# earth-insights/ZoomEarth

Measured on AMD Instinct MI355X. Metric: questions/sec end-to-end, ZoomEarth-3B on 5000px tiles, higher is better.
Workload: dtype bf16

## Files before the change

zoomearth_amd/csrc/ze_attention.hip:

```cpp
#include "ze_kernels.h"

typedef __attribute__((ext_vector_type(8))) __bf16 bf16x8;
typedef __attribute__((ext_vector_type(4))) float f32x4;

#define FA_BQ 64
#ifndef ZE_FA_CAUSAL_BKV
#define ZE_FA_CAUSAL_BKV 64
#endif
#define FA_BK 64

typedef short v4s __attribute__((ext_vector_type(4)));
typedef unsigned int fa_u32x4 __attribute__((ext_vector_type(4)));

__device__ __forceinline__ uint32_t fa_pack_bf16(float lo, float hi) {
    typedef __attribute__((ext_vector_type(2))) float fa_f32x2_;
    typedef __attribute__((ext_vector_type(2))) __bf16 fa_bf16x2_;
    const fa_bf16x2_ b = __builtin_convertvector(fa_f32x2_{lo, hi}, fa_bf16x2_);
    uint32_t r;
    __builtin_memcpy(&r, &b, 4);
    return r;
}

__device__ __forceinline__ int fa_off(int row, int ch) { return 256 * row + 16 * (ch ^ ze_kv_swz(row)); }

template <int D, int CAUSAL, int BKV, int QT = 1, bool DMA = false>
__global__ void __launch_bounds__(256) __attribute__((amdgpu_waves_per_eu(2))) k_flash_attn(const bf16_t* __restrict__ q, int q_rs, int q_hs,
                                                    const bf16_t* __restrict__ k, int k_rs, int k_hs,
                                                    const bf16_t* __restrict__ v, int v_rs, int v_hs,
                                                    bf16_t* __restrict__ o, int o_rs, int o_hs,
                                                    const int4* __restrict__ tiles, int group, float scale_log2e,
                                                    int q_pos_offset, const int* __restrict__ tile_aux,
                                                    size_t kv_seq_stride, ze_fa_rope rope) {
    constexpr int KS = (D + 31) / 32;
    constexpr int DCH = D / 8;
    constexpr int NV = D / 16;
    extern __shared__ __attribute__((aligned(16))) uint8_t smem[];
    constexpr int TILE_B = BKV * 256, NKT = BKV / 16, RP = BKV / 64;

    const int4 tile = tiles[blockIdx.x];
    const int q0 = tile.x, q1 = tile.y, kv0 = tile.z, kv1 = tile.w;
    if (tile_aux) {
        k += (size_t)tile_aux[2 * blockIdx.x] * kv_seq_stride;
        v += (size_t)tile_aux[2 * blockIdx.x] * kv_seq_stride;
        q_pos_offset = tile_aux[2 * blockIdx.x + 1];
    }
    const int head = blockIdx.y, kvh = head / group;
    const int tid = threadIdx.x, lane = tid & 63, wid = tid >> 6;
    const int fr = lane & 15, fq = lane >> 4;
    int qi[QT];
#pragma unroll
    for (int t = 0; t < QT; ++t) qi[t] = q0 + (wid * QT + t) * 16 + fr;

    bf16x8 qf[QT][KS];
#pragma unroll
    for (int t = 0; t < QT; ++t)
#pragma unroll
        for (int ks = 0; ks < KS; ++ks) {
            uint4 val = make_uint4(0, 0, 0, 0);
            const int ch = ks * 4 + fq;
            if (qi[t] < q1 && ch < DCH) val = *reinterpret_cast<const uint4*>(q + (size_t)qi[t] * q_rs + (size_t)head * q_hs + ch * 8);
            qf[t][ks] = *reinterpret_cast<const bf16x8*>(&val);
        }

    f32x4 oacc[QT][NV];
    float m_run[QT], l_run[QT];
#pragma unroll
    for (int t = 0; t < QT; ++t) {
#pragma unroll
        for (int j = 0; j < NV; ++j) oacc[t][j] = f32x4{0.f, 0.f, 0.f, 0.f};
        m_run[t] = -INFINITY;
        l_run[t] = 0.f;
    }
    int kv_hi = kv1;
    if (CAUSAL) kv_hi = min(kv1, q1 + q_pos_offset);
    const int ntile = (kv_hi - kv0 + BKV - 1) / BKV;

    const int srow = tid >> 2, sch = (tid & 3) * 4;
    fa_u32x4 rk[RP][4], rv[RP][4];
    auto stage_load = [&](int kt) {
#pragma unroll
        for (int rp = 0; rp < RP; ++rp) {
            const int keyc = min(kt + rp * 64 + srow, kv_hi - 1);
            const bf16_t* kp = k + (size_t)keyc * k_rs + (size_t)kvh * k_hs;
            const bf16_t* vp = v + (size_t)keyc * v_rs + (size_t)kvh * v_hs;
#pragma unroll
            for (int i = 0; i < 4; ++i) {
                const int ch = min(sch + i, DCH - 1);
                rk[rp][i] = *reinterpret_cast<const fa_u32x4*>(kp + ch * 8);
                rv[rp][i] = *reinterpret_cast<const fa_u32x4*>(vp + ch * 8);
            }
        }
    };
    auto stage_write = [&](int buf, int kt) {
        uint8_t* kb = smem + buf * 2 * TILE_B;
#pragma unroll
        for (int rp = 0; rp < RP; ++rp) {
            const bool ok = kt + rp * 64 + srow < kv_hi;
#pragma unroll
            for (int i = 0; i < 4; ++i) {
                const unsigned m = (ok && (sch + i < DCH)) ? 0xffffffffu : 0u;
                *reinterpret_cast<fa_u32x4*>(kb + fa_off(rp * 64 + srow, sch + i)) = rk[rp][i] & m;
                *reinterpret_cast<fa_u32x4*>(kb + TILE_B + fa_off(rp * 64 + srow, sch + i)) = rv[rp][i] & m;
            }
        }
    };
    static_assert(!DMA || (D == 128 && BKV == 64), "the LDS-DMA staging moves whole 256-byte rows of 64-key tiles");
    const unsigned smem_lds = __builtin_amdgcn_readfirstlane((unsigned)(size_t)(__attribute__((address_space(3))) uint8_t*)smem);
    const int wid_u = __builtin_amdgcn_readfirstlane(wid);
    auto stage_dma = [&](int buf, int kt) {
        const unsigned kimg = smem_lds + (unsigned)buf * 2u * TILE_B, vimg = kimg + TILE_B;
        const int r4 = lane >> 4, pos = lane & 15;
#pragma unroll
        for (int g = 0; g < 4; ++g) {
            const int pc = wid_u * 4 + g;
            const int row = 4 * pc + r4;
            const int ch = pos ^ ze_kv_swz(row);
            const int keyc = min(kt + row, kv_hi - 1);
            const bf16_t* ksrc = k + (size_t)keyc * k_rs + (size_t)kvh * k_hs + ch * 8;
            const bf16_t* vsrc = v + (size_t)keyc * v_rs + (size_t)kvh * v_hs + ch * 8;
            unsigned keep;
            asm volatile(
                "s_mov_b32 %0, m0\n\ts_mov_b32 m0, %3\n\ts_nop 0\n\tglobal_load_lds_dwordx4 %1, off\n\t"
                "s_mov_b32 m0, %4\n\ts_nop 0\n\tglobal_load_lds_dwordx4 %2, off\n\ts_mov_b32 m0, %0"
                : "=&s"(keep)
                : "v"(ksrc), "v"(vsrc), "s"(kimg + (unsigned)pc * 1024u), "s"(vimg + (unsigned)pc * 1024u)
                : "memory");
        }
    };
    if (ntile > 0) {
        if constexpr (DMA) stage_dma(0, kv0);
        else stage_load(kv0);
    }
    if constexpr (D == 128) {
        if (rope.cosT) {
#pragma unroll
            for (int t = 0; t < QT; ++t)
                if (qi[t] < q1) {
#pragma unroll
                    for (int ks = 0; ks < 2; ++ks) {
                        const int j = ks * 32 + fq * 8;
                        const int axis = j < rope.s0 ? 0 : (j < rope.s01 ? 1 : 2);
                        const int pos = rope.pos3[axis * rope.T + qi[t]];
                        const uint4 c4 = *reinterpret_cast<const uint4*>(rope.cosT + (size_t)pos * 64 + j);
                        const uint4 s4 = *reinterpret_cast<const uint4*>(rope.sinT + (size_t)pos * 64 + j);
                        uint4 o1, o2;
                        rope8(*reinterpret_cast<const uint4*>(&qf[t][ks]), *reinterpret_cast<const uint4*>(&qf[t][ks + 2]), c4, s4, o1, o2);
                        qf[t][ks] = *reinterpret_cast<const bf16x8*>(&o1);
                        qf[t][ks + 2] = *reinterpret_cast<const bf16x8*>(&o2);
                    }
                }
        }
    }

    if (ntile > 0) {
        if constexpr (DMA) asm volatile("s_waitcnt vmcnt(0)" ::: "memory");
        else stage_write(0, kv0);
    }
    __syncthreads();

    for (int t = 0; t < ntile; ++t) {
        const int kt = kv0 + t * BKV;
        const uint8_t* kb = smem + (t & 1) * 2 * TILE_B;
        const uint8_t* vb = kb + TILE_B;
        if (t + 1 < ntile) {
            if constexpr (DMA) stage_dma((t + 1) & 1, kt + BKV);
            else stage_load(kt + BKV);
        }
        f32x4 sacc[QT][NKT];
#pragma unroll
        for (int u = 0; u < QT; ++u)
#pragma unroll
            for (int n = 0; n < NKT; ++n) sacc[u][n] = f32x4{0.f, 0.f, 0.f, 0.f};
#pragma unroll
        for (int ks = 0; ks < KS; ++ks) {
#pragma unroll
            for (int n = 0; n < NKT; ++n) {
                const uint4 ka = *reinterpret_cast<const uint4*>(kb + fa_off(n * 16 + fr, ks * 4 + fq));
#pragma unroll
                for (int u = 0; u < QT; ++u)
                    sacc[u][n] = __builtin_amdgcn_mfma_f32_16x16x32_bf16(*reinterpret_cast<const bf16x8*>(&ka), qf[u][ks], sacc[u][n],
                                                                        0, 0, 0);
            }
        }
        uint32_t pw[QT][NKT][2];
#pragma unroll
        for (int u = 0; u < QT; ++u) {
            float p[NKT][4];
// ... 53 lines not shown
                }
            }
#pragma unroll
            for (int n = 0; n < NKT; ++n) {
                pw[u][n][0] = fa_pack_bf16(p[n][0], p[n][1]);
                pw[u][n][1] = fa_pack_bf16(p[n][2], p[n][3]);
            }
        }
#pragma unroll
        for (int ks = 0; ks < BKV / 32; ++ks) {
            bf16x8 pb[QT];
#pragma unroll
            for (int u = 0; u < QT; ++u) {
                const uint4 pq = make_uint4(pw[u][2 * ks][0], pw[u][2 * ks][1], pw[u][2 * ks + 1][0], pw[u][2 * ks + 1][1]);
                pb[u] = *reinterpret_cast<const bf16x8*>(&pq);
            }
#pragma unroll
            for (int j = 0; j < NV; ++j) {
                const int l16 = lane & 15, tq = l16 >> 2, tp = l16 & 3;
                const int r0a = ks * 32 + fq * 4, r0b = r0a + 16;
                const int ch = j * 2 + (tp >> 1), half = 8 * (tp & 1);
                const v4s lo = __builtin_amdgcn_ds_read_tr16_b64_v4i16(
                    (__attribute__((address_space(3))) v4s*)(vb + fa_off(r0a + tq, ch) + half));
                const v4s hi = __builtin_amdgcn_ds_read_tr16_b64_v4i16(
                    (__attribute__((address_space(3))) v4s*)(vb + fa_off(r0b + tq, ch) + half));
                typedef short v8s __attribute__((ext_vector_type(8)));
                const v8s va = __builtin_shufflevector(lo, hi, 0, 1, 2, 3, 4, 5, 6, 7);
#pragma unroll
                for (int u = 0; u < QT; ++u)
                    oacc[u][j] = __builtin_amdgcn_mfma_f32_16x16x32_bf16(*reinterpret_cast<const bf16x8*>(&va), pb[u], oacc[u][j], 0, 0, 0);
            }
        }
        if constexpr (DMA) asm volatile("s_waitcnt vmcnt(0)" ::: "memory");
        else if (t + 1 < ntile) stage_write((t + 1) & 1, kt + BKV);
        __syncthreads();
    }
#pragma unroll
    for (int u = 0; u < QT; ++u)
        if (qi[u] < q1) {
            const float inv = l_run[u] > 0.f ? 1.0f / l_run[u] : 0.f;
#pragma unroll
            for (int j = 0; j < NV; ++j) {
                uint2 w;
                w.x = pack_bf16x2(oacc[u][j][0] * inv, oacc[u][j][1] * inv);
                w.y = pack_bf16x2(oacc[u][j][2] * inv, oacc[u][j][3] * inv);
                *reinterpret_cast<uint2*>(o + (size_t)qi[u] * o_rs + (size_t)head * o_hs + j * 16 + fq * 4) = w;
            }
        }
}

void ze_launch_flash_attn(int D, int causal, const bf16_t* q, int q_rs, int q_hs, const bf16_t* k, int k_rs,
                          int k_hs, const bf16_t* v, int v_rs, int v_hs, bf16_t* o, int o_rs, int o_hs,
                          const int4* tiles, int n_tiles, int heads, int group, float scale, int q_pos_offset,
                          hipStream_t s, const int* tile_aux, size_t kv_seq_stride, int q_tile, int max_kv, ze_fa_rope rope) {
    if (n_tiles == 0) return;
    const float sl = scale * 1.4426950408889634f;
    dim3 grid(n_tiles, heads);
#define FA_LAUNCH_(DD, CC, QQ, DM)                                                                                 \
    do {                                                                                                          \
        constexpr int BKV_ = (CC) ? ZE_FA_CAUSAL_BKV : 64;                                                        \
        constexpr int LDS_ = 4 * BKV_ * 256;                                                                      \
        static bool attr_set = false;                                                                             \
        if (!attr_set) {                                                                                          \
            hipFuncSetAttribute(reinterpret_cast<const void*>(&k_flash_attn<DD, CC, BKV_, QQ, DM>),               \
                                hipFuncAttributeMaxDynamicSharedMemorySize, LDS_);                                \
            attr_set = true;                                                                                      \
        }                                                                                                         \
        const int lds_ = (max_kv > 0 && max_kv <= BKV_) ? LDS_ / 2 : LDS_;                                        \
        hipLaunchKernelGGL((k_flash_attn<DD, CC, BKV_, QQ, DM>), grid, dim3(256), lds_, s, q, q_rs, q_hs, k, k_rs, k_hs, v, v_rs, \
                           v_hs, o, o_rs, o_hs, tiles, group, sl, q_pos_offset, tile_aux, kv_seq_stride, rope);    \
    } while (0)
#define FA_LAUNCH(DD, CC, QQ) FA_LAUNCH_(DD, CC, QQ, false)
    if (D == 128 && causal && ZE_FA_CAUSAL_BKV == 64 && ze_knobs[ZE_KNOB_GATE_UP_FLASH] != ZE_FLASH_REG_STAGED && k_rs % 8 == 0 && v_rs % 8 == 0 && k_hs % 8 == 0 &&
        v_hs % 8 == 0 && ((size_t)k % 16) == 0 && ((size_t)v % 16) == 0 && kv_seq_stride % 8 == 0) {
        if (q_tile > 64) FA_LAUNCH_(128, 1, 2, true);
        else FA_LAUNCH_(128, 1, 1, true);
        return;
    }
    if (q_tile > 64) {
        if (D == 80) {
            if (causal) FA_LAUNCH(80, 1, 2); else FA_LAUNCH(80, 0, 2);
        } else {
            if (causal) FA_LAUNCH(128, 1, 2); else FA_LAUNCH(128, 0, 2);
        }
        return;
    }
    if (D == 80) {
        if (causal) FA_LAUNCH(80, 1, 1); else FA_LAUNCH(80, 0, 1);
    } else {
        if (causal) FA_LAUNCH(128, 1, 1); else FA_LAUNCH(128, 0, 1);
    }
#undef FA_LAUNCH
#undef FA_LAUNCH_
}
```

zoomearth_amd/csrc/ze_elementwise.hip:

```cpp
#include <hip/hip_fp16.h>

#include "ze_kernels.h"
#include "ze_prng.h"
#include "ze_rmsnorm.h"

__device__ __forceinline__ int map_row(int r, int mode, int offset) {
    return mode == 0 ? offset + r : (r >> 4) * 32 + (r & 15) + offset;
}

__global__ void __launch_bounds__(256) k_pack_rows(const void* __restrict__ src, int dtype, int row0, int nrows,
                                                   int cols, bf16_t* __restrict__ dst, int ld, int mode, int offset) {
    const size_t i = (size_t)blockIdx.x * 256 + threadIdx.x;
    if (i >= (size_t)nrows * cols) return;
    const int r = (int)(i / cols), c = (int)(i % cols);
    bf16_t v;
    if (dtype == ZE_BF16) {
        v = ((const bf16_t*)src)[i];
    } else if (dtype == ZE_F16) {
        v = f32_to_bf16(__half2float(((const __half*)src)[i]));
    } else {
        v = f32_to_bf16(((const float*)src)[i]);
    }
    dst[(size_t)map_row(row0 + r, mode, offset) * ld + c] = v;
}

__global__ void __launch_bounds__(256) k_fill_rows(uint64_t seed, float c_scale, float base, int rows, int cols,
                                                   bf16_t* __restrict__ dst, int ld, int mode, int offset) {
    const size_t i = (size_t)blockIdx.x * 256 + threadIdx.x;
    if (i >= (size_t)rows * cols) return;
    const int r = (int)(i / cols), c = (int)(i % cols);
    const float v = (c_scale != 0.0f) ? base + ze_normal_ih4(seed, i, c_scale) : base;
    dst[(size_t)map_row(r, mode, offset) * ld + c] = f32_to_bf16(v);
}

void ze_launch_pack_rows(const void* src, int dtype, int row0, int nrows, int cols, bf16_t* dst, int ld, int mode,
// ... 190 lines not shown
    }
    const uint2 v = *reinterpret_cast<const uint2*>(W + (size_t)row * ld8 + ks * 32 + (lane >> 4) * 8);
    *reinterpret_cast<uint2*>(Wf + (frag * 64 + lane) * 8) = v;
}
void ze_launch_pack_fragments8(const uint8_t* W8, int ld8, int n, int k, uint8_t* Wf8, hipStream_t s, int rope_dim) {
    const size_t frags = (size_t)((n + 15) >> 4) * (k >> 5);
    if (frags == 0) return;
    k_pack_fragments8<<<(unsigned)((frags + 3) / 4), 256, 0, s>>>(W8, ld8, n, k, Wf8, rope_dim);
}

void ze_launch_pack_fragments(const bf16_t* W, int ldw, int n, int k, bf16_t* Wf, hipStream_t s, int rope_dim) {
    const size_t frags = (size_t)((n + 15) >> 4) * (k >> 5);
    if (frags == 0) return;
    k_pack_fragments<<<(unsigned)((frags + 3) / 4), 256, 0, s>>>(W, ldw, n, k, Wf, rope_dim);
}

__global__ void __launch_bounds__(256) k_gather_cast_rows(const float* __restrict__ src, int k,
                                                          const int* __restrict__ perm, bf16_t* __restrict__ dst,
                                                          int kp, int rows) {
    const size_t i = (size_t)blockIdx.x * 256 + threadIdx.x;
    if (i >= (size_t)rows * kp) return;
    const int r = (int)(i / kp), c = (int)(i % kp);
    const int sr = perm ? perm[r] : r;
    dst[i] = c < k ? f32_to_bf16(src[(size_t)sr * k + c]) : (bf16_t)0;
}
void ze_launch_gather_cast_rows(const float* src, int k, const int* perm, bf16_t* dst, int kp, int rows,
                                hipStream_t s) {
    const size_t n = (size_t)rows * kp;
    if (n == 0) return;
    k_gather_cast_rows<<<(unsigned)((n + 255) / 256), 256, 0, s>>>(src, k, perm, dst, kp, rows);
}

__global__ void __launch_bounds__(256) k_vision_rope(bf16_t* __restrict__ qkv, const float* __restrict__ cosT,
                                                     const float* __restrict__ sinT, int n, int heads, int D) {
    const int half = D >> 1;
    const size_t i = (size_t)blockIdx.x * 256 + threadIdx.x;
    const size_t total = (size_t)n * 2 * heads * half;
    if (i >= total) return;
    const int j = (int)(i % half);
    const int hh = (int)((i / half) % heads);
    const int which = (int)((i / ((size_t)half * heads)) % 2);
    const int row = (int)(i / ((size_t)half * heads * 2));
    bf16_t* p = qkv + (((size_t)row * 3 + which) * heads + hh) * D;
    const float c = cosT[(size_t)row * half + j], s = sinT[(size_t)row * half + j];
    const float x1 = bf16_to_f32(p[j]), x2 = bf16_to_f32(p[j + half]);
    p[j] = f32_to_bf16(__fadd_rn(__fmul_rn(x1, c), __fmul_rn(-x2, s)));
    p[j + half] = f32_to_bf16(__fadd_rn(__fmul_rn(x2, c), __fmul_rn(x1, s)));
}
__global__ void __launch_bounds__(256) k_vision_rope_vec(bf16_t* __restrict__ qkv, const float* __restrict__ cosT,
                                                         const float* __restrict__ sinT, int n, int heads, int D) {
    const int half = D >> 1, hv = half >> 3;
    const size_t i = (size_t)blockIdx.x * 256 + threadIdx.x;
    const size_t total = (size_t)n * 2 * heads * hv;
    if (i >= total) return;
    const int j = (int)(i % hv) * 8;
    const int hh = (int)((i / hv) % heads);
    const int which = (int)((i / ((size_t)hv * heads)) % 2);
    const int row = (int)(i / ((size_t)hv * heads * 2));
    bf16_t* p = qkv + (((size_t)row * 3 + which) * heads + hh) * D;
    const uint4 a = *reinterpret_cast<const uint4*>(p + j), b = *reinterpret_cast<const uint4*>(p + j + half);
    const float4 c0 = *reinterpret_cast<const float4*>(cosT + (size_t)row * half + j);
    const float4 c1 = *reinterpret_cast<const float4*>(cosT + (size_t)row * half + j + 4);
    const float4 s0 = *reinterpret_cast<const float4*>(sinT + (size_t)row * half + j);
    const float4 s1 = *reinterpret_cast<const float4*>(sinT + (size_t)row * half + j + 4);
    const float cs[8] = {c0.x, c0.y, c0.z, c0.w, c1.x, c1.y, c1.z, c1.w};
    const float sn[8] = {s0.x, s0.y, s0.z, s0.w, s1.x, s1.y, s1.z, s1.w};
    const uint32_t* pa = reinterpret_cast<const uint32_t*>(&a);
    const uint32_t* pb = reinterpret_cast<const uint32_t*>(&b);
    uint32_t r1[4], r2[4];
#pragma unroll
    for (int q = 0; q < 4; ++q) {
        const float x1l = __uint_as_float(pa[q] << 16), x1h = __uint_as_float(pa[q] & 0xffff0000u);
        const float x2l = __uint_as_float(pb[q] << 16), x2h = __uint_as_float(pb[q] & 0xffff0000u);
        const uint32_t l1 = f32_to_bf16(__fadd_rn(__fmul_rn(x1l, cs[2 * q]), __fmul_rn(-x2l, sn[2 * q])));
        const uint32_t h1 = f32_to_bf16(__fadd_rn(__fmul_rn(x1h, cs[2 * q + 1]), __fmul_rn(-x2h, sn[2 * q + 1])));
        const uint32_t l2 = f32_to_bf16(__fadd_rn(__fmul_rn(x2l, cs[2 * q]), __fmul_rn(x1l, sn[2 * q])));
        const uint32_t h2 = f32_to_bf16(__fadd_rn(__fmul_rn(x2h, cs[2 * q + 1]), __fmul_rn(x1h, sn[2 * q + 1])));
        r1[q] = l1 | (h1 << 16);
        r2[q] = l2 | (h2 << 16);
    }
    *reinterpret_cast<uint4*>(p + j) = make_uint4(r1[0], r1[1], r1[2], r1[3]);
    *reinterpret_cast<uint4*>(p + j + half) = make_uint4(r2[0], r2[1], r2[2], r2[3]);
}
void ze_launch_vision_rope(bf16_t* qkv, const float* cosT, const float* sinT, int n, int heads, int D,
                           hipStream_t s) {
    const size_t total = (size_t)n * 2 * heads * (D / 2);
    if (total == 0) return;
    if ((D / 2) % 8 == 0 && ((size_t)qkv % 16) == 0) {
        const size_t tv = total / 8;
        k_vision_rope_vec<<<(unsigned)((tv + 255) / 256), 256, 0, s>>>(qkv, cosT, sinT, n, heads, D);
        return;
    }
    k_vision_rope<<<(unsigned)((total + 255) / 256), 256, 0, s>>>(qkv, cosT, sinT, n, heads, D);
}

int ze_mrope_vec_ok = 1;
#define mrope_vec_ok (ze_mrope_vec_ok != 0)


__global__ void __launch_bounds__(256) k_mrope_kv(bf16_t* __restrict__ qkv, int T, int heads, int kv_heads, int D,
                                                  const bf16_t* __restrict__ cosT, const bf16_t* __restrict__ sinT,
                                                  const int* __restrict__ pos3, const int* __restrict__ axis_of,
                                                  bf16_t* __restrict__ kcache, bf16_t* __restrict__ vcache,
                                                  int max_ctx, int past, const int* __restrict__ row_aux,
                                                  size_t cache_seq_stride) {
    const int half = D >> 1;
    const int nh = heads + 2 * kv_heads;
    const size_t i = (size_t)blockIdx.x * 256 + threadIdx.x;
    const size_t total = (size_t)T * nh * half;
    if (i >= total) return;
    const int j = (int)(i % half);
    const int hh = (int)((i / half) % nh);
    const int t = (int)(i / ((size_t)half * nh));
    int cpos = past + t;
    if (row_aux) {
        kcache += (size_t)row_aux[2 * t] * cache_seq_stride;
        vcache += (size_t)row_aux[2 * t] * cache_seq_stride;
        cpos = row_aux[2 * t + 1];
    }
    bf16_t* p = qkv + (size_t)t * nh * D + (size_t)hh * D;
    if (hh >= heads + kv_heads) {
        const int kvh = hh - heads - kv_heads;
        bf16_t* d = vcache + ((size_t)kvh * max_ctx + cpos) * D;
        d[j] = p[j];
        d[j + half] = p[j + half];
        return;
// ... 268 lines not shown
```

zoomearth_amd/csrc/ze_kernels.h:

```cpp
#pragma once
#include "ze_common.h"
#include "ze_knobs.h"

enum { ZE_EPI_NONE = 0, ZE_EPI_GELU = 1, ZE_EPI_RESIDUAL = 2, ZE_EPI_SWIGLU = 3, ZE_EPI_F32 = 4, ZE_EPI_QKV_ROPE = 5 };
enum { ZE_GV_QKV_ROPE = 0, ZE_GV_RESIDUAL = 1, ZE_GV_SWIGLU = 2, ZE_GV_LOGITS = 3, ZE_GV_PLAIN = 4 };

#if defined(__HIPCC__)
__device__ __forceinline__ int ze_kv_swz(int row) {
#ifdef ZE_KV_SWZ_OLD
    return ((row & 3) << 2) | ((row >> 2) & 3);
#else
    const int hi = (row >> 3) & 1;
    return ((((row & 7) ^ (hi << 2)) << 1) | hi);
#endif
}
#endif

#if defined(__HIPCC__)
__device__ __forceinline__ void rope8(const uint4& a, const uint4& b, const uint4& c4, const uint4& s4, uint4& o1, uint4& o2) {
    const uint32_t* pa = reinterpret_cast<const uint32_t*>(&a);
    const uint32_t* pb = reinterpret_cast<const uint32_t*>(&b);
    const uint32_t* pc = reinterpret_cast<const uint32_t*>(&c4);
    const uint32_t* ps = reinterpret_cast<const uint32_t*>(&s4);
    uint32_t r1[4], r2[4];
// ... 48 lines not shown
void ze_launch_fill_rows(uint64_t seed, float c_scale, float base, int rows, int cols, bf16_t* dst, int ld, int mode,
                         int offset, hipStream_t s);
struct ze_gemm_ws {
    float* slab = nullptr;
    size_t slab_floats = 0;
    unsigned* tickets = nullptr;
    int ticket_cap = 0;
};
void ze_launch_rmsnorm(const bf16_t* x, int ldx, const bf16_t* w, bf16_t* y, int ldy, int rows, int cols, float eps,
                       hipStream_t s, int frag = 0, int act8 = 0, uint8_t* y8 = nullptr, float* yscale = nullptr);
void ze_launch_pack_fragments(const bf16_t* W, int ldw, int n, int k, bf16_t* Wf, hipStream_t s, int rope_dim = 0);
void ze_launch_gemm_oneshot(int epi, const bf16_t* Xf, const bf16_t* Wf, const bf16_t* bias, const bf16_t* R, int ldr,
                            bf16_t* C, int ldc, int M, int N, int K, hipStream_t s, const float* wscale = nullptr,
                            const float* ascale = nullptr,
                            const uint8_t* wscale4 = nullptr);
void ze_launch_qkv_rope_oneshot(const bf16_t* Xf, const bf16_t* Wf_perm, const bf16_t* bias, bf16_t* q_out, int ldq, int M,
                                int K, int heads, int kv_heads, const bf16_t* cosT, const bf16_t* sinT,
                                const ze_seq_dev* st, const int* seq_ids, bf16_t* kcache, bf16_t* vcache,
                                size_t cache_seq_stride, int max_ctx, hipStream_t s, const float* wscale = nullptr,
                                const float* ascale = nullptr,
                                const int* row_off = nullptr,
                                const uint8_t* wscale4 = nullptr);
bool ze_launch_gemm_mx(int epi, const uint8_t* A, int lda, const float* sa, const uint8_t* W, int ldw, const float* sw,
                       const bf16_t* bias, bf16_t* C, int ldc, int M, int N, int K, hipStream_t s);
void ze_launch_gemm_frag(int epi, const bf16_t* Xf, const bf16_t* Wf, const bf16_t* bias, const bf16_t* R, int ldr,
                         bf16_t* C, int ldc, int M, int N, int K, hipStream_t s, const float* wscale = nullptr,
                         const float* ascale = nullptr,
                         const uint8_t* wscale4 = nullptr);
void ze_launch_pack_fragments8(const uint8_t* W8, int ld8, int n, int k, uint8_t* Wf8, hipStream_t s, int rope_dim = 0);
void ze_launch_pack_fragments4(const uint8_t* q4, const uint8_t* scale, int n, int k, uint8_t* Wf4, uint8_t* Sf4, hipStream_t s,
                               int rope_dim = 0);
void ze_launch_gather_cast_rows(const float* src, int k, const int* perm, bf16_t* dst, int kp, int rows,
                                hipStream_t s);
void ze_launch_vision_rope(bf16_t* qkv, const float* cosT, const float* sinT, int n, int heads, int D, hipStream_t s);
void ze_launch_mrope_kv(bf16_t* qkv, int T, int heads, int kv_heads, int D, const bf16_t* cosT, const bf16_t* sinT,
                        const int* pos3, const int* axis_of, bf16_t* kcache, bf16_t* vcache, int max_ctx, int past, const int* row_aux, size_t cache_seq_stride,
                        hipStream_t s, int q_skip = 0);
extern int ze_mrope_vec_ok;
void ze_launch_embed_rows(const int* src, const bf16_t* embed, const bf16_t* image_embeds, bf16_t* out, int T,
                          int hidden, hipStream_t s);
void ze_launch_scatter_rows(const bf16_t* src, int lds_, const int* dst_idx, bf16_t* dst, int ldd, int rows, int cols,
                            hipStream_t s);

struct ze_qkv_epi {
    const ze_seq_dev* st;
    const int* seq_ids;
    const bf16_t* cosT;
    const bf16_t* sinT;
    bf16_t* kcache;
    bf16_t* vcache;
    size_t cache_seq_stride;
    int max_ctx, heads, kv_heads, pad_;
};
void ze_launch_permute_qkv(const bf16_t* W, int ldw, const bf16_t* bias, int n_heads_total, int K, bf16_t* Wp, bf16_t* bias_p, hipStream_t s);
void ze_launch_gemm_qkv_rope(const bf16_t* A, int lda, const bf16_t* Wp, int ldw, const bf16_t* bias_p, const ze_qkv_epi* dev_args,
                             bf16_t* C, int ldc, int M, int N, int K, hipStream_t s);

void ze_launch_gemm(int epi, const bf16_t* A, int lda, const bf16_t* W, int ldw, const bf16_t* bias, const bf16_t* R,
                    int ldr, bf16_t* C, int ldc, const int* c_rows, int M, int N, int K, hipStream_t s, const ze_gemm_ws& ws = ze_gemm_ws());

void ze_launch_gemm_stream(int epi, const bf16_t* A, int lda, const bf16_t* W, int ldw, const bf16_t* bias,
                           const bf16_t* R, int ldr, bf16_t* C, int ldc, int M, int N, int K, const ze_gemm_ws& ws,
                           hipStream_t s);
void ze_launch_gemm_wide(int epi, const bf16_t* A, int lda, const bf16_t* W, int ldw, const bf16_t* bias, const bf16_t* R,
                         int ldr, bf16_t* C, int ldc, int M, int N, int K, const ze_gemm_ws& ws, hipStream_t s);

void ze_launch_gemm_p8(int epi, const bf16_t* A, int lda, const bf16_t* W, int ldw, const bf16_t* bias, const bf16_t* R, int ldr,
// ... 8 lines not shown
    const bf16_t* bias;
    bf16_t* out_bf16;
    float* out_f32;
    const ze_seq_dev* st;
    const bf16_t* cosT;
    const bf16_t* sinT;
    bf16_t* kcache;
    bf16_t* vcache;
    int heads, kv_heads, D, max_ctx;
    const bf16_t* embed;
    bf16_t* embed_out;
    const uint8_t* W8;
    const float* scale8;
    int ldw8;
    int act8;
    const uint8_t* seen;
    float penalty;
    float* amax_ws;
    const uint8_t* W4;
    const uint8_t* scale4;
};
bool ze_launch_gemv(int epi, const ze_gemv_args& a, hipStream_t s);
bool ze_launch_logits_rows(const bf16_t* W, int ldw, int N, int K, const bf16_t* norm_w, float eps, const bf16_t* const* x_rows,
                           float* const* out_rows, int n, hipStream_t s);
void ze_launch_quantize_rows(bf16_t* w, int rows, int cols, int ld, uint8_t* q, int ld8, float* scale, hipStream_t s);
void ze_launch_quantize_mxfp4(bf16_t* w, int rows, int cols, int ld, uint8_t* q, uint8_t* scale, hipStream_t s);

struct ze_fa_rope {
    const bf16_t* cosT;
    const bf16_t* sinT;
    const int* pos3;
    int s0, s01;
    int T;
};
void ze_launch_flash_attn(int D, int causal, const bf16_t* q, int q_row_stride, int q_head_stride, const bf16_t* k,
                          int k_row_stride, int k_head_stride, const bf16_t* v, int v_row_stride, int v_head_stride,
                          bf16_t* o, int o_row_stride, int o_head_stride, const int4* tiles, int n_tiles, int heads,
                          int group, float scale, int q_pos_offset, hipStream_t s, const int* tile_aux = nullptr,
                          size_t kv_seq_stride = 0, int q_tile = 64, int max_kv = 0, ze_fa_rope rope = ze_fa_rope{nullptr, nullptr, nullptr, 0, 0, 0});
#define ZE_FA_BQ_LONG 128
void ze_launch_attn_decode(const bf16_t* q, int q_row_stride, const bf16_t* kcache, const bf16_t* vcache,
                           size_t cache_seq_stride, bf16_t* out, int out_row_stride, const ze_seq_dev* st,
                           const int* seq_ids, int n, int heads, int kv_heads, int D, int max_ctx, float scale,
                           float* ws_partial, int max_splits, unsigned* tickets, hipStream_t s);

void ze_launch_attn_decode_stream(const bf16_t* q, int q_row_stride, const bf16_t* kcache, const bf16_t* vcache,
                                  size_t cache_seq_stride, bf16_t* out, int out_row_stride, const ze_seq_dev* st,
                                  const int* seq_ids, int n, int heads, int kv_heads, int max_ctx, float scale,
                                  float* ws_partial, int max_parts, unsigned* tickets, hipStream_t s, int chunk = 0,
                                  int per_wave = 0,
                                  const int* prefix = nullptr,
                                  const int* mate = nullptr, int long_parts = 0, int use_split = 0);
void ze_launch_attn_decode_rows(const bf16_t* q, int q_row_stride, const bf16_t* kcache, const bf16_t* vcache, size_t cache_seq_stride,
                                bf16_t* out, int out_row_stride, const ze_seq_dev* st, const int* seq_ids, const int* row_off, int n, int heads,
                                int kv_heads, int max_ctx, float scale, float* ws_partial, unsigned* tickets, int parts, const int* prefix,
                                hipStream_t s);

void ze_launch_kv_copy_prefix(bf16_t* kcache, bf16_t* vcache, size_t layer_stride, size_t seq_stride, size_t head_stride,
                              int layers, int kv_heads, int D, int src, int dst, int n_tokens, hipStream_t s);
void ze_launch_kv_fork(bf16_t* kcache, bf16_t* vcache, size_t layer_stride, size_t seq_stride, size_t head_stride, int layers, int kv_heads,
                       int D, int src, const int* dst_dev, int n, int n_tokens, float* logits, uint8_t* seen, int vocab, hipStream_t s);
int ze_kv_fork_blocks(int runs, int n_vec);
void ze_launch_kv_save(const bf16_t* kcache, const bf16_t* vcache, size_t layer_stride, size_t seq_stride, size_t head_stride, int layers,
                       int kv_heads, int D, int seq, int row0, bf16_t* pool, const int* ids_dev, int nb, int block_rows, hipStream_t s);
void ze_launch_kv_load(bf16_t* kcache, bf16_t* vcache, size_t layer_stride, size_t seq_stride, size_t head_stride, int layers, int kv_heads,
                       int D, const bf16_t* pool, const int* ids_dev, int block_rows, const int* dst_dev, int n, int n_rows, hipStream_t s);
// ... 127 lines not shown
```

zoomearth_amd/csrc/ze_knobs.h:

```cpp
#pragma once

enum ze_knob {
    ZE_KNOB_GEMV_DOWN = 0,
    ZE_KNOB_GATE_UP_FLASH = 1,
    ZE_KNOB_GEMV_GRID_CAP = 2,
    ZE_KNOB_RING32_FROM = 3,
    ZE_KNOB_P8_LAUNCH = 4,
    ZE_KNOB_SKINNY = 5,
    ZE_KNOB_GEMM_STAGING = 6,
    ZE_KNOB_GEMM_TILE = 7,
    ZE_KNOB_BATCH_ATTN = 8,
    ZE_KNOB_O_SKINNY = 9,
    ZE_KNOB_BF16_FRAGMENTS = 10,
    ZE_KNOB_RING_ATTN_PART = 11,
    ZE_KNOB_PREFILL_BF16_GEMM = 12,
    ZE_KNOB_WIDE_DECODE = 13,
    ZE_KNOB_SEPARATE_ARGMAX = 14,
    ZE_KNOB_WIDE_TILES = 15,
    ZE_KNOB_ATTN_ROTATION = 16,
    ZE_KNOB_NO_PREFIX_HINTS = 17,
    ZE_KNOB_KSTEP32 = 18,
    ZE_KNOB_TALL_RING = 19,
    ZE_KNOB_PREFILL_KSPLIT = 20,
    ZE_KNOB_P8_WALK = 21,
    ZE_KNOB_MROPE_Q_IN_PLACE = 22,
    ZE_KNOB_ATTN_SPLIT = 23,
    ZE_KNOB_MX4_BF16_FRAGMENTS = 24,
    ZE_KNOB_COUNT = 25
};
extern int ze_knobs[ZE_KNOB_COUNT];

enum { ZE_KNOB_ON = 1 };
enum { ZE_DOWN_TWO_PAIRS = 1, ZE_DOWN_FOUR_CHUNKS = 2, ZE_DOWN_NO_KSPLIT = 3 };
enum { ZE_GATE_UP_TWO_PAIRS = 1, ZE_GATE_UP_ONE_PAIR = 2, ZE_FLASH_REG_STAGED = 7, ZE_FLASH_BQ64 = 9 };
enum { ZE_P8_TILE_PER_WG = 1, ZE_P8_PERSISTENT = 2 };
enum { ZE_SKINNY_OFF = 1, ZE_SKINNY_GRID32 = 2 };
enum { ZE_STAGING_REGISTERS = 1, ZE_STAGING_RING = 2 };
enum { ZE_TILE_REG_ONLY = 3, ZE_TILE_256 = 4, ZE_TILE_128X256 = 6, ZE_TILE_P8 = 8, ZE_TILE_P8_PER_TILE = 9, ZE_TILE_PLAIN_EPILOGUE = 10 };
enum { ZE_ATTN_SLICE = 1, ZE_ATTN_RING = 2, ZE_ATTN_PLAIN_GRID = 3, ZE_ATTN_PART192 = 4 };
enum { ZE_WIDE_STREAM = 1, ZE_WIDE_QKV_PAIR = 2, ZE_WIDE_TILES_257 = 3, ZE_WIDE_NO_TALL = 4 };
enum { ZE_WT_WSTREAM = 1, ZE_WT_WSTREAM_TILES = 4, ZE_WT_BLOCKS_256 = 5, ZE_WT_ONE_LAUNCH = 6, ZE_WT_NO_TWO_ROW_TILES = 7,
       ZE_WT_WSTREAM_385_512 = 8, ZE_WT_PLAIN = 9 };
enum { ZE_TALL_PLAIN_RING = 4, ZE_PREFILL_KSPLIT_3 = 3 };
enum { ZE_SPLIT_ROWS = 2, ZE_SPLIT_PAIRED = 3 };
```

zoomearth_amd/csrc/ze_vision.hip:

```cpp
#include <math.h>
#include <string.h>

#include "ze_engine.h"

static int frontend_acquire(ze_engine* e) {
    if (e->fe_in_flight) {
        ZE_HIP(hipEventSynchronize(e->fe_done));
        e->fe_in_flight = false;
    }
    return ZE_OK;
}
static int frontend_release(ze_engine* e, hipStream_t s) {
    if (!e->fe_done) ZE_HIP(hipEventCreateWithFlags(&e->fe_done, hipEventDisableTiming));
    ZE_HIP(hipEventRecord(e->fe_done, s));
    e->fe_in_flight = true;
    return ZE_OK;
}

static int crop_resize(ze_engine* e, const uint8_t* src, int src_h, int src_w, const int32_t box[4], uint8_t* dst,
                       int dst_h, int dst_w, hipStream_t s) {
    const int bx0 = box[0], by0 = box[1];
    const int bw = box[2] - box[0], bh = box[3] - box[1];
    if (bw <= 0 || bh <= 0 || dst_w <= 0 || dst_h <= 0) return ze_fail(e, ZE_ERR_INVALID, "empty crop box or output");
    const bool need_h = bw != dst_w, need_v = bh != dst_h;
// ... 207 lines not shown
    int max_win = 0;
    for (size_t i = 1; i < cu_win.size(); ++i) max_win = std::max(max_win, cu_win[i] - cu_win[i - 1]);
    const int bq_full = ze_knobs[ZE_KNOB_GATE_UP_FLASH] == ZE_FLASH_BQ64 ? 64 : ZE_FA_BQ_LONG;
    const int ntf = build_tiles(cu_full.data(), (int)cu_full.size() - 1, tf, n, bq_full);
    if (ntw < 0 || ntf < 0) return ze_fail(e, ZE_ERR_NOMEM, "attention tile list overflow");
    const int nf = half / 2;
    std::vector<float> invf(nf);
    for (int i = 0; i < nf; ++i) invf[i] = 1.0f / powf(10000.0f, (float)(2 * i) / (float)half);
    float* hc = e->v_host_f32;
    float* hs = hc + (size_t)n * half;
    for (int r = 0; r < n; ++r) {
        const int old = perm[r];
        for (int i = 0; i < nf; ++i) {
            const float fh = (float)hw[2 * old] * invf[i], fw = (float)hw[2 * old + 1] * invf[i];
            hc[(size_t)r * half + i] = cosf(fh);
            hs[(size_t)r * half + i] = sinf(fh);
            hc[(size_t)r * half + nf + i] = cosf(fw);
            hs[(size_t)r * half + nf + i] = sinf(fw);
        }
    }
    ZE_HIP(hipMemcpyAsync(e->vperm, perm, (size_t)n * sizeof(int), hipMemcpyHostToDevice, s));
    ZE_HIP(hipMemcpyAsync(e->vinv, inv, (size_t)(n / mu) * sizeof(int), hipMemcpyHostToDevice, s));
    ZE_HIP(hipMemcpyAsync(e->vtiles_win, tw, (size_t)ntw * 16, hipMemcpyHostToDevice, s));
    ZE_HIP(hipMemcpyAsync(e->vtiles_full, tf, (size_t)ntf * 16, hipMemcpyHostToDevice, s));
    ZE_HIP(hipMemcpyAsync(e->vcos, hc, (size_t)n * half * sizeof(float), hipMemcpyHostToDevice, s));
    ZE_HIP(hipMemcpyAsync(e->vsin, hs, (size_t)n * half * sizeof(float), hipMemcpyHostToDevice, s));
    ZE_TRY(stage_release(e, e->v_staged, s));

    const int th = ze_timer_begin(e, 1, s);
    ze_launch_gather_cast_rows(pixel_values, pk, e->vperm, e->vx, pk, n, s);
    ze_launch_gemm(ZE_EPI_NONE, e->vx, pk, e->patch_embed.w, e->patch_embed.ld, nullptr, nullptr, 0, e->vh, vh,
                   nullptr, n, vh, pk, s);
    const float scale = 1.0f / sqrtf((float)hd);
    for (int li = 0; li < c.vit_depth; ++li) {
        const ze_vit_block& b = e->vb[li];
        bool full = false;
        for (int k = 0; k < c.n_fullatt; ++k) full |= c.fullatt_block_indexes[k] == li;
        ze_launch_rmsnorm(e->vh, vh, b.norm1, e->vy, vh, n, vh, 1e-6f, s);
        ze_launch_gemm(ZE_EPI_NONE, e->vy, vh, b.qkv.w, b.qkv.ld, b.qkv.bias, nullptr, 0, e->vqkv, 3 * vh, nullptr, n,
                       3 * vh, vh, s);
        ze_launch_vision_rope(e->vqkv, e->vcos, e->vsin, n, nh, hd, s);
        ze_launch_flash_attn(hd, 0, e->vqkv, 3 * vh, hd, e->vqkv + vh, 3 * vh, hd, e->vqkv + 2 * vh, 3 * vh, hd, e->vo,
                             vh, hd, full ? e->vtiles_full : e->vtiles_win, full ? ntf : ntw, nh, 1, scale, 0, s, nullptr, 0,
                             full ? bq_full : 64, full ? 0 : max_win);
        ze_launch_gemm(ZE_EPI_RESIDUAL, e->vo, vh, b.proj.w, b.proj.ld, b.proj.bias, e->vh, vh, e->vh, vh, nullptr, n,
                       vh, vh, s);
        ze_launch_rmsnorm(e->vh, vh, b.norm2, e->vy, vh, n, vh, 1e-6f, s);
        ze_launch_gemm(ZE_EPI_SWIGLU, e->vy, vh, b.gate_up.w, b.gate_up.ld, b.gate_up.bias, nullptr, 0, e->va,
                       e->vit_ipad, nullptr, n, 2 * e->vit_ipad, vh, s);
        ze_launch_gemm(ZE_EPI_RESIDUAL, e->va, e->vit_ipad, b.down.w, b.down.ld, b.down.bias, e->vh, vh, e->vh, vh,
                       nullptr, n, vh, e->vit_ipad, s);
    }
    ze_launch_rmsnorm(e->vh, vh, e->ln_q, e->vy, vh, n, vh, 1e-6f, s);
    const int mh = vh * mu;
    ze_launch_gemm(ZE_EPI_GELU, e->vy, mh, e->merger0.w, e->merger0.ld, e->merger0.bias, nullptr, 0, e->vz, mh, nullptr,
                   n / mu, mh, mh, s);
    ze_launch_gemm(ZE_EPI_NONE, e->vz, mh, e->merger2.w, e->merger2.ld, e->merger2.bias, nullptr, 0,
                   (bf16_t*)out_embeds, c.vit_out_hidden, e->vinv, n / mu, c.vit_out_hidden, mh, s);
    ze_timer_end(e, th, s);
    ZE_KCHECK();
    return ZE_OK;
}
```

Baseline: 69.56.

## Fold ViT 2D rotary embedding into flash-attention Q/K loads

Adds a rotate-on-load path to the D=80 non-causal flash-attention kernel that applies vision RoPE to Q in registers and to K while staging tiles into LDS, using per-row cos/sin tables. Windowed ViT blocks skip the standalone rope kernel entirely; full-attention blocks still pre-rotate K in a K-only pass and rotate Q on load. This removes a read-modify-write pass over Q/K in global memory and a kernel launch per layer, at the cost of extra table loads, register pressure and redundant K rotation across query tiles inside attention. It also changes the rounding slightly, since the shared helper now uses an FMA.

```diff
diff --git a/zoomearth_amd/csrc/ze_attention.hip b/zoomearth_amd/csrc/ze_attention.hip
--- a/zoomearth_amd/csrc/ze_attention.hip
+++ b/zoomearth_amd/csrc/ze_attention.hip
@@ -1,4 +1,5 @@
 #include "ze_kernels.h"
+#include "ze_vision_rope.h"
 
 typedef __attribute__((ext_vector_type(8))) __bf16 bf16x8;
 typedef __attribute__((ext_vector_type(4))) float f32x4;
@@ -23,7 +24,7 @@
 
 __device__ __forceinline__ int fa_off(int row, int ch) { return 256 * row + 16 * (ch ^ ze_kv_swz(row)); }
 
-template <int D, int CAUSAL, int BKV, int QT = 1, bool DMA = false>
+template <int D, int CAUSAL, int BKV, int QT = 1, bool DMA = false, int VR = 0>
 __global__ void __launch_bounds__(256) __attribute__((amdgpu_waves_per_eu(2))) k_flash_attn(const bf16_t* __restrict__ q, int q_rs, int q_hs,
                                                     const bf16_t* __restrict__ k, int k_rs, int k_hs,
                                                     const bf16_t* __restrict__ v, int v_rs, int v_hs,
@@ -76,7 +77,17 @@
     const int ntile = (kv_hi - kv0 + BKV - 1) / BKV;
 
     const int srow = tid >> 2, sch = (tid & 3) * 4;
+    static_assert(VR == 0 || (D == 80 && !DMA), "rotate-on-load is the ViT's: D = 80 (five 16-byte chunks per half), register staging");
+    auto slot_ch = [&](int i) -> int {
+        if constexpr (VR == 1) {
+            const int c = tid & 3;
+            return i == 0 ? c : (i == 1 ? c + DCH / 2 : (c == 0 ? (i == 2 ? DCH / 2 - 1 : DCH - 1) : DCH - 4 + 2 * c + i));
+        } else {
+            return sch + i;
+        }
+    };
     fa_u32x4 rk[RP][4], rv[RP][4];
+    float4 rc[VR == 1 ? RP : 1][2][4];
     auto stage_load = [&](int kt) {
 #pragma unroll
         for (int rp = 0; rp < RP; ++rp) {
@@ -85,9 +96,25 @@
             const bf16_t* vp = v + (size_t)keyc * v_rs + (size_t)kvh * v_hs;
 #pragma unroll
             for (int i = 0; i < 4; ++i) {
-                const int ch = min(sch + i, DCH - 1);
+                const int ch = min(slot_ch(i), DCH - 1);
                 rk[rp][i] = *reinterpret_cast<const fa_u32x4*>(kp + ch * 8);
                 rv[rp][i] = *reinterpret_cast<const fa_u32x4*>(vp + ch * 8);
+            }
+        }
+    };
+    auto stage_load_tables = [&](int kt) {
+        if constexpr (VR == 1) {
+#pragma unroll
+            for (int rp = 0; rp < RP; ++rp) {
+                const int keyc = min(kt + rp * 64 + srow, kv_hi - 1);
+#pragma unroll
+                for (int pr = 0; pr < 2; ++pr) {
+                    const size_t at = (size_t)keyc * (D / 2) + (pr == 0 ? (tid & 3) : DCH / 2 - 1) * 8;
+                    rc[rp][pr][0] = *reinterpret_cast<const float4*>(rope.vcos + at);
+                    rc[rp][pr][1] = *reinterpret_cast<const float4*>(rope.vcos + at + 4);
+                    rc[rp][pr][2] = *reinterpret_cast<const float4*>(rope.vsin + at);
+                    rc[rp][pr][3] = *reinterpret_cast<const float4*>(rope.vsin + at + 4);
+                }
             }
         }
     };
@@ -96,11 +123,23 @@
 #pragma unroll
         for (int rp = 0; rp < RP; ++rp) {
             const bool ok = kt + rp * 64 + srow < kv_hi;
+            if constexpr (VR == 1) {
+#pragma unroll
+                for (int pr = 0; pr < 2; ++pr) {
+                    uint4 a, b, o1, o2;
+                    __builtin_memcpy(&a, &rk[rp][2 * pr], 16);
+                    __builtin_memcpy(&b, &rk[rp][2 * pr + 1], 16);
+                    ze_vrope8(a, b, rc[rp][pr][0], rc[rp][pr][1], rc[rp][pr][2], rc[rp][pr][3], o1, o2);
+                    __builtin_memcpy(&rk[rp][2 * pr], &o1, 16);
+                    __builtin_memcpy(&rk[rp][2 * pr + 1], &o2, 16);
+                }
+            }
 #pragma unroll
             for (int i = 0; i < 4; ++i) {
-                const unsigned m = (ok && (sch + i < DCH)) ? 0xffffffffu : 0u;
-                *reinterpret_cast<fa_u32x4*>(kb + fa_off(rp * 64 + srow, sch + i)) = rk[rp][i] & m;
-                *reinterpret_cast<fa_u32x4*>(kb + TILE_B + fa_off(rp * 64 + srow, sch + i)) = rv[rp][i] & m;
+                const int ch = slot_ch(i);
+                const unsigned m = (ok && (ch < DCH)) ? 0xffffffffu : 0u;
+                *reinterpret_cast<fa_u32x4*>(kb + fa_off(rp * 64 + srow, ch)) = rk[rp][i] & m;
+                *reinterpret_cast<fa_u32x4*>(kb + TILE_B + fa_off(rp * 64 + srow, ch)) = rv[rp][i] & m;
             }
         }
     };
@@ -151,8 +190,32 @@
                 }
         }
     }
+    if constexpr (VR != 0) {
+#pragma unroll
+        for (int t = 0; t < QT; ++t) {
+            const int qr = min(qi[t], q1 - 1);
+            const bf16_t* qp = q + (size_t)qr * q_rs + (size_t)head * q_hs;
+            const float* cr = rope.vcos + (size_t)qr * (D / 2);
+            const float* sr = rope.vsin + (size_t)qr * (D / 2);
+#pragma unroll
+            for (int ks = 0; ks < KS; ++ks) {
+                const int ch = min(ks * 4 + fq, DCH - 1);
+                const bool lo = ch < DCH / 2;
+                const int j = (lo ? ch : ch - DCH / 2) * 8;
+                uint4 own, oth = *reinterpret_cast<const uint4*>(qp + (lo ? ch + DCH / 2 : ch - DCH / 2) * 8), o1, o2;
+                __builtin_memcpy(&own, &qf[t][ks], 16);
+                const float4 c0 = *reinterpret_cast<const float4*>(cr + j), c1 = *reinterpret_cast<const float4*>(cr + j + 4);
+                const float4 s0 = *reinterpret_cast<const float4*>(sr + j), s1 = *reinterpret_cast<const float4*>(sr + j + 4);
+                ze_vrope8(lo ? own : oth, lo ? oth : own, c0, c1, s0, s1, o1, o2);
+                uint4 r = lo ? o1 : o2;
+                if (qi[t] >= q1 || ks * 4 + fq >= DCH) r = make_uint4(0, 0, 0, 0);
+                __builtin_memcpy(&qf[t][ks], &r, 16);
+            }
+        }
+    }
 
     if (ntile > 0) {
+        stage_load_tables(kv0);
         if constexpr (DMA) asm volatile("s_waitcnt vmcnt(0)" ::: "memory");
         else stage_write(0, kv0);
     }
@@ -272,7 +335,10 @@
             }
         }
         if constexpr (DMA) asm volatile("s_waitcnt vmcnt(0)" ::: "memory");
-        else if (t + 1 < ntile) stage_write((t + 1) & 1, kt + BKV);
+        else if (t + 1 < ntile) {
+            stage_load_tables(kt + BKV);
+            stage_write((t + 1) & 1, kt + BKV);
+        }
         __syncthreads();
     }
 #pragma unroll
@@ -296,25 +362,38 @@
     if (n_tiles == 0) return;
     const float sl = scale * 1.4426950408889634f;
     dim3 grid(n_tiles, heads);
-#define FA_LAUNCH_(DD, CC, QQ, DM)                                                                                 \
+#define FA_LAUNCH_(DD, CC, QQ, DM, VV)                                                                             \
     do {                                                                                                          \
         constexpr int BKV_ = (CC) ? ZE_FA_CAUSAL_BKV : 64;                                                        \
         constexpr int LDS_ = 4 * BKV_ * 256;                                                                      \
         static bool attr_set = false;                                                                             \
         if (!attr_set) {                                                                                          \
-            hipFuncSetAttribute(reinterpret_cast<const void*>(&k_flash_attn<DD, CC, BKV_, QQ, DM>),               \
+            hipFuncSetAttribute(reinterpret_cast<const void*>(&k_flash_attn<DD, CC, BKV_, QQ, DM, VV>),           \
                                 hipFuncAttributeMaxDynamicSharedMemorySize, LDS_);                                \
             attr_set = true;                                                                                      \
         }                                                                                                         \
         const int lds_ = (max_kv > 0 && max_kv <= BKV_) ? LDS_ / 2 : LDS_;                                        \
-        hipLaunchKernelGGL((k_flash_attn<DD, CC, BKV_, QQ, DM>), grid, dim3(256), lds_, s, q, q_rs, q_hs, k, k_rs, k_hs, v, v_rs, \
+        hipLaunchKernelGGL((k_flash_attn<DD, CC, BKV_, QQ, DM, VV>), grid, dim3(256), lds_, s, q, q_rs, q_hs, k, k_rs, k_hs, v, v_rs, \
                            v_hs, o, o_rs, o_hs, tiles, group, sl, q_pos_offset, tile_aux, kv_seq_stride, rope);    \
     } while (0)
-#define FA_LAUNCH(DD, CC, QQ) FA_LAUNCH_(DD, CC, QQ, false)
+#define FA_LAUNCH(DD, CC, QQ) FA_LAUNCH_(DD, CC, QQ, false, 0)
+    if (rope.vcos) {
+        if (D != 80 || causal || !rope.vsin || !ze_vision_rope_vec_ok(q, D) || !ze_vision_rope_vec_ok(k, D) || q_rs % 8 || q_hs % 8 ||
+            k_rs % 8 || k_hs % 8) {
+            fprintf(stderr, "ze_launch_flash_attn: rotate-on-load needs the non-causal D = 80 kernel on 16-byte aligned rows\n");
+            abort();
+        }
+        if (q_tile > 64) {
+            if (rope.fold_k) FA_LAUNCH_(80, 0, 2, false, 1); else FA_LAUNCH_(80, 0, 2, false, 2);
+        } else {
+            if (rope.fold_k) FA_LAUNCH_(80, 0, 1, false, 1); else FA_LAUNCH_(80, 0, 1, false, 2);
+        }
+        return;
+    }
     if (D == 128 && causal && ZE_FA_CAUSAL_BKV == 64 && ze_knobs[ZE_KNOB_GATE_UP_FLASH] != ZE_FLASH_REG_STAGED && k_rs % 8 == 0 && v_rs % 8 == 0 && k_hs % 8 == 0 &&
         v_hs % 8 == 0 && ((size_t)k % 16) == 0 && ((size_t)v % 16) == 0 && kv_seq_stride % 8 == 0) {
-        if (q_tile > 64) FA_LAUNCH_(128, 1, 2, true);
-        else FA_LAUNCH_(128, 1, 1, true);
+        if (q_tile > 64) FA_LAUNCH_(128, 1, 2, true, 0);
+        else FA_LAUNCH_(128, 1, 1, true, 0);
         return;
     }
     if (q_tile > 64) {
diff --git a/zoomearth_amd/csrc/ze_elementwise.hip b/zoomearth_amd/csrc/ze_elementwise.hip
--- a/zoomearth_amd/csrc/ze_elementwise.hip
+++ b/zoomearth_amd/csrc/ze_elementwise.hip
@@ -1,6 +1,7 @@
 #include <hip/hip_fp16.h>
 
 #include "ze_kernels.h"
+#include "ze_vision_rope.h"
 #include "ze_prng.h"
 #include "ze_rmsnorm.h"
 
@@ -257,15 +258,15 @@
 }
 
 __global__ void __launch_bounds__(256) k_vision_rope(bf16_t* __restrict__ qkv, const float* __restrict__ cosT,
-                                                     const float* __restrict__ sinT, int n, int heads, int D) {
+                                                     const float* __restrict__ sinT, int n, int heads, int D, int first, int count) {
     const int half = D >> 1;
     const size_t i = (size_t)blockIdx.x * 256 + threadIdx.x;
-    const size_t total = (size_t)n * 2 * heads * half;
+    const size_t total = (size_t)n * count * heads * half;
     if (i >= total) return;
     const int j = (int)(i % half);
     const int hh = (int)((i / half) % heads);
-    const int which = (int)((i / ((size_t)half * heads)) % 2);
-    const int row = (int)(i / ((size_t)half * heads * 2));
+    const int which = first + (int)((i / ((size_t)half * heads)) % count);
+    const int row = (int)(i / ((size_t)half * heads * count));
     bf16_t* p = qkv + (((size_t)row * 3 + which) * heads + hh) * D;
     const float c = cosT[(size_t)row * half + j], s = sinT[(size_t)row * half + j];
     const float x1 = bf16_to_f32(p[j]), x2 = bf16_to_f32(p[j + half]);
@@ -273,50 +274,37 @@
     p[j + half] = f32_to_bf16(__fadd_rn(__fmul_rn(x2, c), __fmul_rn(x1, s)));
 }
 __global__ void __launch_bounds__(256) k_vision_rope_vec(bf16_t* __restrict__ qkv, const float* __restrict__ cosT,
-                                                         const float* __restrict__ sinT, int n, int heads, int D) {
+                                                         const float* __restrict__ sinT, int n, int heads, int D, int first, int count) {
     const int half = D >> 1, hv = half >> 3;
     const size_t i = (size_t)blockIdx.x * 256 + threadIdx.x;
-    const size_t total = (size_t)n * 2 * heads * hv;
+    const size_t total = (size_t)n * count * heads * hv;
     if (i >= total) return;
     const int j = (int)(i % hv) * 8;
     const int hh = (int)((i / hv) % heads);
-    const int which = (int)((i / ((size_t)hv * heads)) % 2);
-    const int row = (int)(i / ((size_t)hv * heads * 2));
+    const int which = first + (int)((i / ((size_t)hv * heads)) % count);
+    const int row = (int)(i / ((size_t)hv * heads * count));
     bf16_t* p = qkv + (((size_t)row * 3 + which) * heads + hh) * D;
     const uint4 a = *reinterpret_cast<const uint4*>(p + j), b = *reinterpret_cast<const uint4*>(p + j + half);
     const float4 c0 = *reinterpret_cast<const float4*>(cosT + (size_t)row * half + j);
     const float4 c1 = *reinterpret_cast<const float4*>(cosT + (size_t)row * half + j + 4);
     const float4 s0 = *reinterpret_cast<const float4*>(sinT + (size_t)row * half + j);
     const float4 s1 = *reinterpret_cast<const float4*>(sinT + (size_t)row * half + j + 4);
-    const float cs[8] = {c0.x, c0.y, c0.z, c0.w, c1.x, c1.y, c1.z, c1.w};
-    const float sn[8] = {s0.x, s0.y, s0.z, s0.w, s1.x, s1.y, s1.z, s1.w};
-    const uint32_t* pa = reinterpret_cast<const uint32_t*>(&a);
-    const uint32_t* pb = reinterpret_cast<const uint32_t*>(&b);
-    uint32_t r1[4], r2[4];
-#pragma unroll
-    for (int q = 0; q < 4; ++q) {
-        const float x1l = __uint_as_float(pa[q] << 16), x1h = __uint_as_float(pa[q] & 0xffff0000u);
-        const float x2l = __uint_as_float(pb[q] << 16), x2h = __uint_as_float(pb[q] & 0xffff0000u);
-        const uint32_t l1 = f32_to_bf16(__fadd_rn(__fmul_rn(x1l, cs[2 * q]), __fmul_rn(-x2l, sn[2 * q])));
-        const uint32_t h1 = f32_to_bf16(__fadd_rn(__fmul_rn(x1h, cs[2 * q + 1]), __fmul_rn(-x2h, sn[2 * q + 1])));
-        const uint32_t l2 = f32_to_bf16(__fadd_rn(__fmul_rn(x2l, cs[2 * q]), __fmul_rn(x1l, sn[2 * q])));
-        const uint32_t h2 = f32_to_bf16(__fadd_rn(__fmul_rn(x2h, cs[2 * q + 1]), __fmul_rn(x1h, sn[2 * q + 1])));
-        r1[q] = l1 | (h1 << 16);
-        r2[q] = l2 | (h2 << 16);
-    }
-    *reinterpret_cast<uint4*>(p + j) = make_uint4(r1[0], r1[1], r1[2], r1[3]);
-    *reinterpret_cast<uint4*>(p + j + half) = make_uint4(r2[0], r2[1], r2[2], r2[3]);
+    uint4 o1, o2;
+    ze_vrope8(a, b, c0, c1, s0, s1, o1, o2);
+    *reinterpret_cast<uint4*>(p + j) = o1;
+    *reinterpret_cast<uint4*>(p + j + half) = o2;
 }
 void ze_launch_vision_rope(bf16_t* qkv, const float* cosT, const float* sinT, int n, int heads, int D,
-                           hipStream_t s) {
-    const size_t total = (size_t)n * 2 * heads * (D / 2);
+                           hipStream_t s, int k_only) {
+    const int first = k_only ? 1 : 0, count = k_only ? 1 : 2;
+    const size_t total = (size_t)n * count * heads * (D / 2);
     if (total == 0) return;
-    if ((D / 2) % 8 == 0 && ((size_t)qkv % 16) == 0) {
+    if (ze_vision_rope_vec_ok(qkv, D)) {
         const size_t tv = total / 8;
-        k_vision_rope_vec<<<(unsigned)((tv + 255) / 256), 256, 0, s>>>(qkv, cosT, sinT, n, heads, D);
-        return;
-    }
-    k_vision_rope<<<(unsigned)((total + 255) / 256), 256, 0, s>>>(qkv, cosT, sinT, n, heads, D);
+        k_vision_rope_vec<<<(unsigned)((tv + 255) / 256), 256, 0, s>>>(qkv, cosT, sinT, n, heads, D, first, count);
+        return;
+    }
+    k_vision_rope<<<(unsigned)((total + 255) / 256), 256, 0, s>>>(qkv, cosT, sinT, n, heads, D, first, count);
 }
 
 int ze_mrope_vec_ok = 1;
diff --git a/zoomearth_amd/csrc/ze_kernels.h b/zoomearth_amd/csrc/ze_kernels.h
--- a/zoomearth_amd/csrc/ze_kernels.h
+++ b/zoomearth_amd/csrc/ze_kernels.h
@@ -104,7 +104,8 @@
                                int rope_dim = 0);
 void ze_launch_gather_cast_rows(const float* src, int k, const int* perm, bf16_t* dst, int kp, int rows,
                                 hipStream_t s);
-void ze_launch_vision_rope(bf16_t* qkv, const float* cosT, const float* sinT, int n, int heads, int D, hipStream_t s);
+void ze_launch_vision_rope(bf16_t* qkv, const float* cosT, const float* sinT, int n, int heads, int D, hipStream_t s, int k_only = 0);
+inline bool ze_vision_rope_vec_ok(const bf16_t* qkv, int D) { return (D / 2) % 8 == 0 && ((size_t)qkv % 16) == 0; }
 void ze_launch_mrope_kv(bf16_t* qkv, int T, int heads, int kv_heads, int D, const bf16_t* cosT, const bf16_t* sinT,
                         const int* pos3, const int* axis_of, bf16_t* kcache, bf16_t* vcache, int max_ctx, int past, const int* row_aux, size_t cache_seq_stride,
                         hipStream_t s, int q_skip = 0);
@@ -179,6 +180,9 @@
     const int* pos3;
     int s0, s01;
     int T;
+    const float* vcos;
+    const float* vsin;
+    int fold_k;
 };
 void ze_launch_flash_attn(int D, int causal, const bf16_t* q, int q_row_stride, int q_head_stride, const bf16_t* k,
                           int k_row_stride, int k_head_stride, const bf16_t* v, int v_row_stride, int v_head_stride,
diff --git a/zoomearth_amd/csrc/ze_knobs.h b/zoomearth_amd/csrc/ze_knobs.h
--- a/zoomearth_amd/csrc/ze_knobs.h
+++ b/zoomearth_amd/csrc/ze_knobs.h
@@ -32,7 +32,9 @@
 
 enum { ZE_KNOB_ON = 1 };
 enum { ZE_DOWN_TWO_PAIRS = 1, ZE_DOWN_FOUR_CHUNKS = 2, ZE_DOWN_NO_KSPLIT = 3 };
-enum { ZE_GATE_UP_TWO_PAIRS = 1, ZE_GATE_UP_ONE_PAIR = 2, ZE_FLASH_REG_STAGED = 7, ZE_FLASH_BQ64 = 9 };
+enum { ZE_GATE_UP_TWO_PAIRS = 1, ZE_GATE_UP_ONE_PAIR = 2, ZE_FLASH_REG_STAGED = 7, ZE_FLASH_BQ64 = 9,
+       ZE_FLASH_VIT_ROPE_PASS = 10,
+       ZE_FLASH_VIT_ROPE_PASS_FULL_BLOCKS = 11 };
 enum { ZE_P8_TILE_PER_WG = 1, ZE_P8_PERSISTENT = 2 };
 enum { ZE_SKINNY_OFF = 1, ZE_SKINNY_GRID32 = 2 };
 enum { ZE_STAGING_REGISTERS = 1, ZE_STAGING_RING = 2 };
diff --git a/zoomearth_amd/csrc/ze_vision.hip b/zoomearth_amd/csrc/ze_vision.hip
--- a/zoomearth_amd/csrc/ze_vision.hip
+++ b/zoomearth_amd/csrc/ze_vision.hip
@@ -263,6 +263,8 @@
     ze_launch_gemm(ZE_EPI_NONE, e->vx, pk, e->patch_embed.w, e->patch_embed.ld, nullptr, nullptr, 0, e->vh, vh,
                    nullptr, n, vh, pk, s);
     const float scale = 1.0f / sqrtf((float)hd);
+    const int rope_knob = ze_knobs[ZE_KNOB_GATE_UP_FLASH];
+    const bool can_fold = hd == 80 && ze_vision_rope_vec_ok(e->vqkv, hd) && vh % 8 == 0 && rope_knob != ZE_FLASH_VIT_ROPE_PASS;
     for (int li = 0; li < c.vit_depth; ++li) {
         const ze_vit_block& b = e->vb[li];
         bool full = false;
@@ -270,10 +272,17 @@
         ze_launch_rmsnorm(e->vh, vh, b.norm1, e->vy, vh, n, vh, 1e-6f, s);
         ze_launch_gemm(ZE_EPI_NONE, e->vy, vh, b.qkv.w, b.qkv.ld, b.qkv.bias, nullptr, 0, e->vqkv, 3 * vh, nullptr, n,
                        3 * vh, vh, s);
-        ze_launch_vision_rope(e->vqkv, e->vcos, e->vsin, n, nh, hd, s);
+        const bool fold = can_fold && !(full && rope_knob == ZE_FLASH_VIT_ROPE_PASS_FULL_BLOCKS);
+        ze_fa_rope rope{nullptr, nullptr, nullptr, 0, 0, 0};
+        if (fold) {
+            rope.vcos = e->vcos;
+            rope.vsin = e->vsin;
+            rope.fold_k = full ? 0 : 1;
+        }
+        if (!fold || full) ze_launch_vision_rope(e->vqkv, e->vcos, e->vsin, n, nh, hd, s, fold ? 1 : 0);
         ze_launch_flash_attn(hd, 0, e->vqkv, 3 * vh, hd, e->vqkv + vh, 3 * vh, hd, e->vqkv + 2 * vh, 3 * vh, hd, e->vo,
                              vh, hd, full ? e->vtiles_full : e->vtiles_win, full ? ntf : ntw, nh, 1, scale, 0, s, nullptr, 0,
-                             full ? bq_full : 64, full ? 0 : max_win);
+                             full ? bq_full : 64, full ? 0 : max_win, rope);
         ze_launch_gemm(ZE_EPI_RESIDUAL, e->vo, vh, b.proj.w, b.proj.ld, b.proj.bias, e->vh, vh, e->vh, vh, nullptr, n,
                        vh, vh, s);
         ze_launch_rmsnorm(e->vh, vh, b.norm2, e->vy, vh, n, vh, 1e-6f, s);
diff --git a/zoomearth_amd/csrc/ze_vision_rope.h b/zoomearth_amd/csrc/ze_vision_rope.h
--- /dev/null
+++ b/zoomearth_amd/csrc/ze_vision_rope.h
@@ -0,0 +1,28 @@
+#pragma once
+#include "ze_common.h"
+
+#if defined(__HIPCC__)
+__device__ __forceinline__ void ze_vrope_pair(float x1, float x2, float c, float s, float& o1, float& o2) {
+    o1 = __fmaf_rn(x1, c, -__fmul_rn(x2, s));
+    o2 = __fmaf_rn(x1, s, __fmul_rn(x2, c));
+}
+
+__device__ __forceinline__ void ze_vrope8(const uint4& a, const uint4& b, const float4& c0, const float4& c1, const float4& s0,
+                                          const float4& s1, uint4& o1, uint4& o2) {
+    const float cs[8] = {c0.x, c0.y, c0.z, c0.w, c1.x, c1.y, c1.z, c1.w};
+    const float sn[8] = {s0.x, s0.y, s0.z, s0.w, s1.x, s1.y, s1.z, s1.w};
+    const uint32_t* pa = reinterpret_cast<const uint32_t*>(&a);
+    const uint32_t* pb = reinterpret_cast<const uint32_t*>(&b);
+    uint32_t r1[4], r2[4];
+#pragma unroll
+    for (int q = 0; q < 4; ++q) {
+        float l1, l2, h1, h2;
+        ze_vrope_pair(bf16lo(pa[q]), bf16lo(pb[q]), cs[2 * q], sn[2 * q], l1, l2);
+        ze_vrope_pair(bf16hi(pa[q]), bf16hi(pb[q]), cs[2 * q + 1], sn[2 * q + 1], h1, h2);
+        r1[q] = pack_bf16x2(l1, h1);
+        r2[q] = pack_bf16x2(l2, h2);
+    }
+    o1 = make_uint4(r1[0], r1[1], r1[2], r1[3]);
+    o2 = make_uint4(r2[0], r2[1], r2[2], r2[3]);
+}
+#endif
```

New measurement: 69.83 (median of 2 runs). No clear change (+0.4%).
